# Wulizhou888/3DGS-RayTrace

Measured on AMD Instinct MI355X. Metric: Mrays/s @1080p, 1M Gaussians; achieved HBM GB/s vs peak; 1→8 GPU scaling, higher is better.
Workload: dtype f32; 1 GPU; c3: 1000000 Gaussians SH-3, 1920x1080, 4 spp, COR; gaussians=1000000, width=1920, height=1080, spp=4, sh_degree=3, parallelism=1 GPU

## Files before the change

3dgs-raytrace_amd/csrc/gsrt_render.hip:

```cpp
#include <algorithm>
#include <cmath>
#include <cstdlib>
#include <cstring>
#include <vector>
#include <type_traits>

#include "gsrt_internal.hpp"
#include "gsrt_project.hpp"

namespace gsrt {

constexpr uint32_t kStack = 512;
constexpr uint32_t kGroup = 4;
constexpr uint32_t kRCap = 128;
constexpr uint32_t kRBuf = 2 * kRCap;
constexpr uint32_t kRStack = 256;
constexpr uint32_t kGCap = 896;
#ifndef GSRT_GROUP_SEGMENTS
#define GSRT_GROUP_SEGMENTS 2
#endif
constexpr uint32_t kGSegs = GSRT_GROUP_SEGMENTS;
constexpr uint32_t kGStride = kGSegs * kGCap;
constexpr uint32_t kMoreLanes = 16;
constexpr uint32_t kGBuf = 1024;
// ... 547 lines not shown

__device__ GSRT_INLINE void add_counters(unsigned long long rays, unsigned long long cand, unsigned long long blended,
                                    unsigned long long term, unsigned long long rounds, unsigned long long restarts,
                                    unsigned long long maxc) {
    if (lane_id() != 0) return;
    unsigned long long* c = kargs().a.counters;
    atomicAdd(c + 0, rays);
    atomicAdd(c + 1, cand);
    atomicAdd(c + 2, blended);
    atomicAdd(c + 3, term);
    atomicAdd(c + 4, rounds);
    atomicAdd(c + 5, restarts);
    atomicAdd(c + 6, 1ull);
    atomicMax(c + 7, maxc);
}


struct Stage {
    SplatRec rec[kGroup];
    float sh[kGroup][3][16];
};
static_assert(sizeof(Stage) == kGroup * 256 && sizeof(Stage) % 1024 == 0, "whole wave-instructions of 16-B pieces");

template <uint32_t N>
__device__ GSRT_INLINE void wait_vmcnt() { asm volatile("s_waitcnt vmcnt(%0)" ::"n"(N) : "memory"); }
template <class V>
__device__ GSRT_INLINE void wait_stage(uint32_t younger) {
    constexpr uint32_t P = V::stage_ops;
    if (younger >= 2) wait_vmcnt<2 * P>();
    else if (younger == 1) wait_vmcnt<P>();
    else wait_vmcnt<0>();
}

__device__ GSRT_INLINE uint32_t lds_read_settled(const uint32_t* p) {
    const uint32_t a = (uint32_t)(uintptr_t)(const __attribute__((address_space(3))) uint32_t*)p;
    uint32_t v;
    asm volatile("ds_read_b32 %0, %1\n\ts_waitcnt lgkmcnt(0)" : "=v"(v) : "v"(a) : "memory");
    return v;
}

template <class V>
__device__ GSRT_INLINE void stage_issue(const uint32_t* ids, uint32_t count, uint32_t g0, uint32_t lane, Stage* dst,
                                   const SplatRec* recs, const float* sh) {
    constexpr uint32_t kRecPieces = 4 * kGroup, kPieces = V::stage_pieces, kRowPieces = V::row_pieces;
#pragma unroll
    for (uint32_t i = 0; i < (kPieces + 63) / 64; ++i) {
        const uint32_t p = i * 64 + lane;
        const bool is_rec = p < kRecPieces;
        const uint32_t q = p - kRecPieces;
        uint32_t c = g0 + (is_rec ? p >> 2 : q / kRowPieces);
        c = c < count ? c : g0;
        if (p < kPieces) {
            const uint32_t id = lds_read_settled(ids + c);
            const char* base = is_rec ? reinterpret_cast<const char*>(recs) : reinterpret_cast<const char*>(sh);
            const uint32_t stride = is_rec ? 64u : kRowPieces * 16u, off = is_rec ? (p & 3) * 16u : (q % kRowPieces) * 16u;
            __builtin_amdgcn_global_load_lds((const void*)(base + (size_t)id * stride + off),
                                             (void*)(reinterpret_cast<char*>(dst) + i * 1024), 16, 0, 0);
        }
    }
}

__device__ GSRT_INLINE void list_issue(uint32_t lt, uint32_t lane, uint32_t* ids, uint32_t* hdr) {
    const KArgs& K = kargs();
    const uint32_t* src = K.a.lists + (size_t)lt * kCap;
    __builtin_amdgcn_global_load_lds((const void*)(src + lane), (void*)ids, 4, 0, 0);
    __builtin_amdgcn_global_load_lds((const void*)(src + 64 + lane), (void*)(ids + 64), 4, 0, 0);
    if (lane < 4)
        __builtin_amdgcn_global_load_lds((const void*)(reinterpret_cast<const uint32_t*>(K.a.list_hdr + lt) + lane),
                                         (void*)hdr, 4, 0, 0);
}

template <class V>
struct CorRay {
    ObjRay R;
    float pxs, pys;
    float bs[16];
    float T, C[3];
    typename V::RayPayload k;
    bool active;
    uint32_t cand, blended, term;
#ifdef GSRT_DIAG
    uint32_t dg_staged, dg_gpass, dg_contrib, dg_blend, dg_lanes_g, dg_lanes_blend;
    uint32_t dg_stages, dg_stages_blend, dg_lane_max;
#endif
};

__device__ GSRT_INLINE float sh_channel(const float (&bs)[16], const float (&s)[16]) {
    float a = s[0];
#pragma unroll
    for (int q = 1; q < 16; ++q) a = fmaf(bs[q], s[q], a);
    return a > 0.0f ? a : 0.0f;
}
struct ShFromStage {
    const Stage* stg;
    uint32_t c;
    __device__ GSRT_INLINE void operator()(const float (&bs)[16], float (&col)[3]) const {
#pragma unroll
        for (int ch = 0; ch < 3; ++ch) {
            const float4* s4 = reinterpret_cast<const float4*>(stg->sh[c][ch]);
            const float4 q0 = s4[0], q1 = s4[1], q2 = s4[2], q3 = s4[3];
            const float s[16] = {q0.x, q0.y, q0.z, q0.w, q1.x, q1.y, q1.z, q1.w,
                                 q2.x, q2.y, q2.z, q2.w, q3.x, q3.y, q3.z, q3.w};
            col[ch] = sh_channel(bs, s);
        }
    }
};
__device__ GSRT_INLINE bool lane_of(uint64_t mask) { return __builtin_amdgcn_inverse_ballot_w64(mask); }
__device__ GSRT_INLINE const float4* feat_row(const Stage* stg, uint32_t c) {
    return reinterpret_cast<const float4*>(&stg->sh[0][0][0]) + 4 * c;
}
template <int CTRL>
__device__ GSRT_INLINE float dpp_from(float v) {
    return __int_as_float(__builtin_amdgcn_mov_dpp(__float_as_int(v), CTRL, 0xF, 0xF, false));
}
__device__ GSRT_INLINE float grad_row_sums(const float (&t)[16]) {
    const bool b3 = lane_of(0xFF00FF00FF00FF00ull), b2 = lane_of(0xF0F0F0F0F0F0F0F0ull);
    const bool b1 = lane_of(0xCCCCCCCCCCCCCCCCull), b0 = lane_of(0xAAAAAAAAAAAAAAAAull);
    float a[8], b[4], c[2];
#pragma unroll
    for (int k = 0; k < 8; ++k) a[k] = (b3 ? t[8 + k] : t[k]) + dpp_from<0x140>(b3 ? t[k] : t[8 + k]);
#pragma unroll
    for (int k = 0; k < 4; ++k) b[k] = (b2 ? a[4 + k] : a[k]) + dpp_from<0x141>(b2 ? a[k] : a[4 + k]);
#pragma unroll
    for (int k = 0; k < 2; ++k) c[k] = (b1 ? b[2 + k] : b[k]) + dpp_from<0x4E>(b1 ? b[k] : b[2 + k]);
    return (b0 ? c[1] : c[0]) + dpp_from<0xB1>(b0 ? c[0] : c[1]);
}
__device__ GSRT_INLINE float grad_stage_sums(const float (&gs)[kGroup]) {
    static_assert(kGroup == 4, "one candidate per 16-lane row");
    typedef uint32_t u32x2 __attribute__((ext_vector_type(2)));
    const u32x2 p = __builtin_amdgcn_permlane32_swap(__float_as_uint(gs[0]), __float_as_uint(gs[2]), false, false);
    const u32x2 q = __builtin_amdgcn_permlane32_swap(__float_as_uint(gs[1]), __float_as_uint(gs[3]), false, false);
    const float u = __uint_as_float(p.x) + __uint_as_float(p.y);
    const float v = __uint_as_float(q.x) + __uint_as_float(q.y);
    const u32x2 r = __builtin_amdgcn_permlane16_swap(__float_as_uint(u), __float_as_uint(v), false, false);
    return __uint_as_float(r.x) + __uint_as_float(r.y);
}
__device__ GSRT_INLINE float opgrad_stage_sums(const float (&t)[kGroup]) {
    static_assert(kGroup == 4, "one candidate per lane of a quad");
    typedef uint32_t u32x2 __attribute__((ext_vector_type(2)));
    const bool b1 = lane_of(0xCCCCCCCCCCCCCCCCull), b0 = lane_of(0xAAAAAAAAAAAAAAAAull);
    float c[2];
#pragma unroll
    for (int k = 0; k < 2; ++k) c[k] = (b1 ? t[2 + k] : t[k]) + dpp_from<0x4E>(b1 ? t[k] : t[2 + k]);
    float v = (b0 ? c[1] : c[0]) + dpp_from<0xB1>(b0 ? c[0] : c[1]);
    v = v + dpp_from<0x128>(v);
    v = v + dpp_from<0x124>(v);
    const u32x2 p = __builtin_amdgcn_permlane16_swap(__float_as_uint(v), __float_as_uint(v), false, false);
    const float u = __uint_as_float(p.x) + __uint_as_float(p.y);
    const u32x2 q = __builtin_amdgcn_permlane32_swap(__float_as_uint(u), __float_as_uint(u), false, false);
    return __uint_as_float(q.x) + __uint_as_float(q.y);
}
__device__ GSRT_INLINE float over_samples(float x, uint32_t ns) {
    const float nsf = (float)ns;
    return (ns & (ns - 1)) == 0 ? x * (1.0f / nsf) : x / nsf;
}

template <int N>
__device__ GSRT_INLINE void load_upstream(float (&G)[N], uint32_t x, uint32_t y, bool valid, uint32_t ns) {
    const KArgs& K = kargs();
    const float* gi = K.a.grad_in + ((size_t)y * K.a.width + x) * 4;
#pragma unroll
    for (int q = 0; q < N; ++q) G[q] = valid ? over_samples(gi[q], ns) : 0.0f;
}
template <uint32_t PER, class Sums, class Add>
__device__ GSRT_INLINE void flush_share(const uint32_t* ids, uint32_t mask, Sums sums, Add add) {
    const auto sum = sums();
// ... 133 lines not shown
        }
        __device__ GSRT_INLINE void flush() const {
            flush_share<1>(ids, mask, [&] { return opgrad_stage_sums(t); },
                           [&](uint32_t id, uint32_t, float sum) { atomicAdd(rows + id, sum); });
        }
    };
    __device__ GSRT_INLINE Share share(const uint32_t* ids) const { return Share{ids, rows}; }
};

enum class CorKind { plain, stats, depth, feat, grad, shgrad, opgrad };
constexpr uint32_t kFeatWaves = 4;
constexpr uint32_t kGradWaves = GSRT_GRAD_WAVES;
constexpr uint32_t kShGradWaves = GSRT_SHGRAD_WAVES;
constexpr uint32_t kOpGradWaves = GSRT_OPGRAD_WAVES;
struct NoPayload {};
struct DepthPayload { float D; };
struct ChannelPayload { float F[16]; };
template <CorKind K, bool SH, bool LUT>
struct CorVariant {
    static constexpr bool sh = SH, lut = LUT;
    static constexpr bool stats = K == CorKind::stats, depth = K == CorKind::depth;
    static constexpr bool feat = K == CorKind::feat, grad = K == CorKind::grad, shgrad = K == CorKind::shgrad;
    static constexpr bool opgrad = K == CorKind::opgrad;
    static_assert(!(feat || grad) || !SH, "feature and gradient frames evaluate no SH");
    static_assert(!shgrad || SH, "an SH gradient frame blends the SH rows");
    static constexpr uint32_t waves =
        opgrad ? kOpGradWaves : shgrad ? kShGradWaves : grad ? kGradWaves : feat ? kFeatWaves
        : SH ? (LUT ? (K == CorKind::plain ? 5 : 4) : 6) : (LUT ? 5 : 6);
    static constexpr uint32_t row_pieces = feat ? 4u : 12u;
    static constexpr uint32_t stage_pieces = SH ? 16 * kGroup : (feat ? 8 * kGroup : 4 * kGroup);
    static constexpr uint32_t stage_ops = (stage_pieces + 63) / 64;
    using Grad = std::conditional_t<grad, FeatureGrad, std::conditional_t<shgrad, ShGrad,
                                    std::conditional_t<opgrad, OpacityGrad, NoGrad>>>;
    using SumPayload = std::conditional_t<depth, DepthPayload, std::conditional_t<feat, ChannelPayload, NoPayload>>;
    using RayPayload = std::conditional_t<std::is_same_v<Grad, NoGrad>, SumPayload, typename Grad::Payload>;
};
template <class V, class Sh>
__device__ GSRT_INLINE uint64_t blend_hit(const Stage* stg, uint32_t c, float z, float alpha, uint64_t contrib,
                                          CorRay<V>& ray, Sh& grad) {
    const float tn = ray.T * (1.0f - alpha);
    const uint64_t low = __ballot(tn < 1e-4f);
    const uint64_t term = contrib & low;
    const uint64_t blend = contrib & ~low;
    if (blend) {
        float col[3] = {1.0f, 1.0f, 1.0f};
        if (V::sh) ShFromStage{stg, c}(ray.bs, col);
        grad.hit(c, blend, alpha, col, ray);
        if (lane_of(blend)) {
            const float w = alpha * ray.T;
            ray.C[0] = fmaf(col[0], w, ray.C[0]);
            if constexpr (!V::feat && !V::grad) {
                ray.C[1] = fmaf(col[1], w, ray.C[1]);
                ray.C[2] = fmaf(col[2], w, ray.C[2]);
            }
            if constexpr (V::depth) ray.k.D = fmaf(z, w, ray.k.D);
            if constexpr (V::feat) {
                const float4* frow = feat_row(stg, c);
#pragma unroll
                for (int q = 0; q < 4; ++q) {
                    const float4 f = frow[q];
                    ray.k.F[4 * q + 0] = fmaf(f.x, w, ray.k.F[4 * q + 0]);
                    ray.k.F[4 * q + 1] = fmaf(f.y, w, ray.k.F[4 * q + 1]);
                    ray.k.F[4 * q + 2] = fmaf(f.z, w, ray.k.F[4 * q + 2]);
                    ray.k.F[4 * q + 3] = fmaf(f.w, w, ray.k.F[4 * q + 3]);
                }
            }
            grad.hit_lane(c, alpha, col, ray);
            ray.T = tn;
            if (V::stats) ++ray.blended;
        }
    }
    if (term) {
        if (lane_of(term)) {
            ray.active = false;
            ray.pxs = __builtin_nanf("");
            if (V::stats) ++ray.term;
        }
    }
    return term;
}

template <class V>
constexpr bool kShPerLane = V::sh && !V::stats && !V::shgrad && !V::opgrad;
struct StageBlends {
    uint64_t blend[kGroup] = {0, 0, 0, 0};
    float w[kGroup] = {0.0f, 0.0f, 0.0f, 0.0f};
};
template <class V>
__device__ GSRT_INLINE uint64_t weigh_hit(uint32_t c, float alpha, uint64_t contrib, CorRay<V>& ray, StageBlends& sb) {
    const float tn = ray.T * (1.0f - alpha);
    const uint64_t low = __ballot(tn < 1e-4f);
    const uint64_t term = contrib & low;
    const uint64_t blend = contrib & ~low;
    sb.blend[c] = blend;
    sb.w[c] = alpha * ray.T;
    ray.T = lane_of(blend) ? tn : ray.T;
    if (term) {
        if (lane_of(term)) {
            ray.active = false;
            ray.pxs = __builtin_nanf("");
        }
    }
    return term;
}
template <class V, uint32_t J>
__device__ GSRT_INLINE bool blend_pass(const Stage* stg, const uint64_t (&at)[kGroup][kGroup], const float (&ws)[kGroup],
                                       CorRay<V>& ray) {
    uint64_t any = at[J][J];
    if constexpr (J + 1 < kGroup) any |= at[J][J + 1];
    if constexpr (J + 2 < kGroup) any |= at[J][J + 2];
    if constexpr (J + 3 < kGroup) any |= at[J][J + 3];
    if (!any) return false;
#ifdef GSRT_DIAG
    ray.dg_lane_max += 1u;
#endif
    if (lane_of(any)) {
        uint32_t cj = J;
        float w = ws[J];
        if constexpr (J + 1 < kGroup) {
            const bool here = lane_of(at[J][J + 1]);
            cj = here ? J + 1 : cj, w = here ? ws[J + 1] : w;
        }
        if constexpr (J + 2 < kGroup) {
            const bool here = lane_of(at[J][J + 2]);
            cj = here ? J + 2 : cj, w = here ? ws[J + 2] : w;
        }
        if constexpr (J + 3 < kGroup) {
            const bool here = lane_of(at[J][J + 3]);
            cj = here ? J + 3 : cj, w = here ? ws[J + 3] : w;
        }
        float col[3];
        ShFromStage{stg, cj}(ray.bs, col);
        ray.C[0] = fmaf(col[0], w, ray.C[0]);
        ray.C[1] = fmaf(col[1], w, ray.C[1]);
        ray.C[2] = fmaf(col[2], w, ray.C[2]);
        if constexpr (V::depth) ray.k.D = fmaf(stg->rec[cj].depth, w, ray.k.D);
    }
    return true;
}
template <class V>
__device__ GSRT_INLINE void blend_stage(const Stage* stg, const StageBlends& sb, CorRay<V>& ray) {
    static_assert(kGroup == 4, "two bit planes count a lane's earlier blends; blend_pass selects among four");
    if (!(sb.blend[0] | sb.blend[1] | sb.blend[2] | sb.blend[3])) return;
#ifdef GSRT_DIAG
    ray.dg_stages_blend += 1u;
#endif
    uint64_t at[kGroup][kGroup];
    uint64_t p0 = 0, p1 = 0;
#pragma unroll
    for (uint32_t c = 0; c < kGroup; ++c) {
        const uint64_t b = sb.blend[c];
        at[0][c] = b & ~p0 & ~p1;
        at[1][c] = b & p0 & ~p1;
        at[2][c] = b & ~p0 & p1;
        at[3][c] = b & p0 & p1;
        const uint64_t carry = p0 & b;
        p0 ^= b;
        p1 ^= carry;
    }
    float ws[kGroup] = {sb.w[0], sb.w[1], sb.w[2], sb.w[3]};
    asm volatile("" : "+v"(ws[0]), "+v"(ws[1]), "+v"(ws[2]), "+v"(ws[3]));
    if (!blend_pass<V, 0>(stg, at, ws, ray)) return;
    if (!blend_pass<V, 1>(stg, at, ws, ray)) return;
    if (!blend_pass<V, 2>(stg, at, ws, ray)) return;
    blend_pass<V, 3>(stg, at, ws, ray);
}

template <class V, bool FULL, class Sh>
__device__ GSRT_INLINE void shade_stage(const Stage* stg, uint32_t m, const float* lut_s, CorRay<V>& ray, Sh grad) {
    constexpr bool LUT = V::lut;
    if constexpr (!V::stats) {
        float gv[kGroup];
        uint64_t okg[kGroup];
#pragma unroll
        for (uint32_t c = 0; c < kGroup; ++c) {
            const float4 q2 = reinterpret_cast<const float4*>(&stg->rec[c])[2];
            float4 q3 = reinterpret_cast<const float4*>(&stg->rec[c])[3];
            asm volatile("" : "+v"(q3.w));
            const float c2 = q3.x, cut = LUT ? kGMax : q3.y;
            const float dx = ray.pxs - q2.x, dy = ray.pys - q2.y;
            gv[c] = fmaf(c2 * dy, dy, fmaf(q2.w * dx, dy, (q2.z * dx) * dx));
            okg[c] = (FULL || c < m) ? __ballot(__float_as_uint(gv[c]) <= __float_as_uint(cut)) : 0;
        }
#ifdef GSRT_DIAG
        ray.dg_staged += __ballot(ray.active) ? m : 0u;
        ray.dg_stages += __ballot(ray.active) ? 1u : 0u;
#endif
        [[maybe_unused]] StageBlends sb;
#pragma unroll
        for (uint32_t c = 0; c < kGroup; ++c) {
            if (!okg[c]) continue;
            float4 q0 = reinterpret_cast<const float4*>(&stg->rec[c])[0];
            const float4 q1 = reinterpret_cast<const float4*>(&stg->rec[c])[1];
            asm volatile("" : "+v"(q0.w));
            const float lo[3] = {q0.x, q0.y, q0.z}, hi[3] = {q1.x, q1.y, q1.z};
            const bool ordered = (int)__builtin_amdgcn_readfirstlane(__float_as_uint(q1.w)) >= 0;
            const uint64_t ok = okg[c] & (ordered ? __ballot(slab_hit_ordered(ray.R, lo, hi))
                                                  : __ballot(slab_hit_rel(ray.R, lo, hi)));
            const float gs = LUT ? (lane_of(ok) ? gv[c] : 0.0f) : gv[c];
            const float e = LUT ? linear_exp(lut_s, gs) : exp_neg_nocheck(-gs);
            const float a = __builtin_fminf(fabsf(q1.w) * e, 0.99f);
            const uint64_t contrib = ok & __ballot(a > kAlphaMin);
            const float alpha = lane_of(contrib) ? a : 0.0f;
#ifdef GSRT_DIAG
            ray.dg_gpass += 1u;
            ray.dg_lanes_g += (uint32_t)__popcll(okg[c]);
            ray.dg_contrib += __ballot(alpha > 0.0f) ? 1u : 0u;
            ray.dg_blend += __ballot(alpha > 0.0f && ray.T * (1.0f - alpha) >= 1e-4f) ? 1u : 0u;
            ray.dg_lanes_blend += (uint32_t)__popcll(__ballot(alpha > 0.0f && ray.T * (1.0f - alpha) >= 1e-4f));
#endif
            grad.candidate(e, fabsf(q1.w));
            uint64_t stopped;
            if constexpr (kShPerLane<V>) stopped = weigh_hit<V>(c, alpha, contrib, ray, sb);
            else stopped = blend_hit<V>(stg, c, q0.w, alpha, contrib, ray, grad);
            if (stopped) {
#pragma unroll
                for (uint32_t c1 = c + 1; c1 < kGroup; ++c1) okg[c1] &= ~stopped;
            }
        }
        if constexpr (kShPerLane<V>) blend_stage<V>(stg, sb, ray);
        if (grad.mask) grad.flush();
    } else {
        for (uint32_t c = 0; c < m; ++c) {
            const float4* r4 = reinterpret_cast<const float4*>(&stg->rec[c]);
            float4 q0 = r4[0], q1 = r4[1], q2 = r4[2], q3 = r4[3];
            asm volatile("" : "+v"(q1.w), "+v"(q2.x), "+v"(q2.y), "+v"(q2.z), "+v"(q2.w), "+v"(q3.x), "+v"(q3.z));
            float alpha = 0.0f;
            if (ray.active) {
                const float lo[3] = {q0.x, q0.y, q0.z}, hi[3] = {q1.x, q1.y, q1.z};
                if (slab_hit_rel(ray.R, lo, hi)) {
                    ++ray.cand;
                    const float dx = ray.pxs - q2.x, dy = ray.pys - q2.y;
                    const float g = fmaf(q3.x * dy, dy, fmaf(q2.w * dx, dy, (q2.z * dx) * dx));
                    if (g >= 0.0f && g <= kGMax) {
                        const float e = LUT ? linear_exp(lut_s, g) : exp_neg(-g);
                        float a = fabsf(q1.w) * e;
                        if (a > 0.99f) a = 0.99f;
                        if (a > kAlphaMin) alpha = a;
                    }
                }
            }
            blend_hit<V>(stg, c, q0.w, alpha, __ballot(alpha > 0.0f), ray, grad);
        }
    }
}


template <class V, class S>
__device__ GSRT_INLINE bool shade_sorted(const uint32_t* ids, uint32_t count, Stage* stA, Stage* stB, Stage* stC,
                             const float* lut_s, CorRay<V>& ray, const SplatRec* recs, const float* sh, S sink) {
    const uint32_t lane = lane_id();
    count = __builtin_amdgcn_readfirstlane(count);
    if (count == 0) return __ballot(ray.active) != 0;
    auto issue = [&](uint32_t g, Stage* dst) { stage_issue<V>(ids, count, g, lane, dst, recs, sh); };
    auto shade = [&](Stage* stg, uint32_t g) {
        const uint32_t m = count - g < kGroup ? count - g : kGroup;
        shade_stage<V, false>(stg, m, lut_s, ray, sink.share(ids + g));
    };
    auto shade_full = [&](Stage* stg, uint32_t g) {
        shade_stage<V, true>(stg, kGroup, lut_s, ray, sink.share(ids + g));
    };
    constexpr uint32_t kWaitTwo = 2 * V::stage_ops;
    auto wait = [count](uint32_t g) {
        wait_stage<V>((g + kGroup < count ? 1u : 0u) + (g + 2 * kGroup < count ? 1u : 0u));
    };
    issue(0, stA);
    if (kGroup < count) issue(kGroup, stB);
    bool live = true;
    uint32_t g0 = 0;
    if (!V::stats) {
        for (; g0 + 4 * kGroup < count; g0 += 3 * kGroup) {
            issue(g0 + 2 * kGroup, stC);
            wait_vmcnt<kWaitTwo>();
            shade_full(stA, g0);
            if (!__ballot(ray.active)) { live = false; break; }
            issue(g0 + 3 * kGroup, stA);
            wait_vmcnt<kWaitTwo>();
            shade_full(stB, g0 + kGroup);
            if (!__ballot(ray.active)) { live = false; break; }
            issue(g0 + 4 * kGroup, stB);
            wait_vmcnt<kWaitTwo>();
            shade_full(stC, g0 + 2 * kGroup);
            if (!__ballot(ray.active)) { live = false; break; }
        }
    }
    for (; live && g0 < count; g0 += 3 * kGroup) {
        if (g0 + 2 * kGroup < count) issue(g0 + 2 * kGroup, stC);
        wait(g0);
        shade(stA, g0);
        if (!__ballot(ray.active)) { live = false; break; }
        const uint32_t g1 = g0 + kGroup;
        if (g1 >= count) break;
        if (g1 + 2 * kGroup < count) issue(g1 + 2 * kGroup, stA);
        wait(g1);
        shade(stB, g1);
        if (!__ballot(ray.active)) { live = false; break; }
        const uint32_t g2 = g1 + kGroup;
        if (g2 >= count) break;
        if (g2 + 2 * kGroup < count) issue(g2 + 2 * kGroup, stB);
        wait(g2);
        shade(stC, g2);
        if (!__ballot(ray.active)) { live = false; break; }
    }
// ... 409 lines not shown
        p.valid = p.x < kargs().a.width && p.y < kargs().a.height;
        return p;
    }
    __device__ GSRT_INLINE TileRect rect_here() const {
        uint32_t tx = x0 >> lgtw, ty = y0 >> lgth;
        asm volatile("" : "+s"(tx), "+s"(ty));
        return tile_rect(tx, ty, tw, th);
    }
};

template <class V>
struct PixelSums {
    float rgba[4];
    typename V::SumPayload k;
    template <class Op>
    __device__ GSRT_INLINE void each(Op op) {
#pragma unroll
        for (int q = 0; q < 4; ++q) op(rgba[q]);
        if constexpr (V::depth) op(k.D);
        if constexpr (V::feat) {
#pragma unroll
            for (int q = 0; q < 16; ++q) op(k.F[q]);
        }
    }
    template <class Op>
    __device__ GSRT_INLINE void each_extra_at(size_t pix, Op op) {
        if constexpr (V::depth) op(k.D, kargs().a.depth_out + pix);
        if constexpr (V::feat) {
            const uint32_t C = kargs().a.feat_channels;
            float* of = kargs().a.feat_out + pix * C;
#pragma unroll
            for (int q = 0; q < 16; ++q)
                if ((uint32_t)q < C) op(k.F[q], of + q);
        }
    }
    template <class Op>
    __device__ GSRT_INLINE void each_at(float* colour, size_t pix, Op op) {
#pragma unroll
        for (int q = 0; q < 4; ++q) op(rgba[q], colour + q);
        each_extra_at(pix, op);
    }
    __device__ GSRT_INLINE void take(const CorRay<V>& ray) {
        constexpr bool grey = V::feat || V::grad;
        rgba[0] = ray.C[0]; rgba[1] = ray.C[grey ? 0 : 1]; rgba[2] = ray.C[grey ? 0 : 2]; rgba[3] = 1.0f - ray.T;
        if constexpr (V::depth) k.D = ray.k.D;
        if constexpr (V::feat) {
#pragma unroll
            for (int q = 0; q < 16; ++q) k.F[q] = ray.k.F[q];
        }
    }
};

template <class V>
__device__ GSRT_INLINE CorRay<V> cor_ray(const CorTile::Pixel& p, uint32_t S, uint32_t pass, uint32_t passes) {
    CorRay<V> ray;
    {
        const KArgs& K = kargs();
        const uint32_t sidx = pass * S + p.s;
        uint32_t seed = K.ubo.random_seed;
        for (uint32_t q = 0; q < sidx; ++q) { random_float(&seed); random_float(&seed); }
        const float jx = random_float(&seed);
        const float jy = random_float(&seed);
        ray.pxs = (float)p.x + jx;
        ray.pys = (float)p.y + jy;
        float o[3], d[3];
        gen_ray(K.ubo, ray.pxs, ray.pys, o, d);
        ray.R = make_obj_ray(d);
        if (V::sh) sh_basis(d, ray.bs);
    }
    ray.T = 1.0f;
    ray.C[0] = ray.C[1] = ray.C[2] = 0.0f;
    if constexpr (V::depth) ray.k.D = 0.0f;
    if constexpr (V::feat) {
#pragma unroll
        for (int q = 0; q < 16; ++q) ray.k.F[q] = 0.0f;
    }
    V::Grad::load(ray.k, p.x, p.y, p.valid, S * passes);
    ray.active = p.valid;
    if (!p.valid) ray.pxs = __builtin_nanf("");
    ray.cand = ray.blended = ray.term = 0;
#ifdef GSRT_DIAG
    ray.dg_staged = ray.dg_gpass = ray.dg_contrib = ray.dg_blend = ray.dg_lanes_g = ray.dg_lanes_blend = 0;
    ray.dg_stages = ray.dg_stages_blend = ray.dg_lane_max = 0;
#endif
    return ray;
}

__device__ GSRT_INLINE Collected round_from_list(const CorTile& t, bool& prefetched, uint32_t* ids, const uint32_t* lhdr,
                                                 uint64_t& lo, uint32_t& gpos) {
    Collected cl{};
    if (!prefetched) list_issue(t.lt, lane_here(), ids, const_cast<uint32_t*>(lhdr));
    prefetched = false;
    __syncthreads();
    const uint4 h = make_uint4(lhdr[0], lhdr[1], lhdr[2], lhdr[3]);
    const uint32_t* src = kargs().a.lists + (size_t)t.lt * kCap;
    cl.count = h.x & 0x7fffffffu;
    cl.more = (h.x >> 31) != 0;
    for (uint32_t i = 128u + lane_here(); i < cl.count; i += 64) ids[i] = src[i];
    cl.total = cl.count;
    lo = ((uint64_t)h.w << 32) | h.z;
    gpos = h.y;
    __syncthreads();
    return cl;
}
__device__ GSRT_INLINE Collected round_from_group(const CorTile& t, uint32_t* ids, uint64_t& lo, uint32_t& gpos, bool& found) {
    Collected cl{};
    const KArgs& K = kargs();
    const uint32_t g = (t.y0 / t.th / K.a.fg) * K.a.groups_x + (t.x0 / t.tw / K.a.fg);
    const uint4 gh = K.a.ghdr[g];
    const uint32_t gcount = gh.x & 0x7fffffffu;
    found = gpos < gcount;
    if (!found) return cl;
    const uint64_t* gl = K.a.glist + (size_t)g * kGStride;
    const float4* fps = K.a.footprint;
    const TileRect rect_c = t.rect_here();
    uint32_t out = 0;
    while (gpos < gcount && out < kCap) {
        const uint32_t i = gpos + lane_here();
        bool keep = false;
        uint64_t key = 0;
        if (i < gcount) {
            key = gl[i];
            keep = fp_meets(fps, (uint32_t)key, rect_c);
        }
        const uint64_t b = __ballot(keep);
        const uint32_t rank = popc_below(b), n = (uint32_t)__popcll(b), room = kCap - out;
        if (keep && rank < room) ids[out + rank] = (uint32_t)key;
        if (n > room) {
            const uint64_t kb = __ballot(keep && rank < room);
            gpos += (uint32_t)(63 - __builtin_clzll(kb)) + 1u;
            out = kCap;
        } else {
            gpos = gpos + 64u < gcount ? gpos + 64u : gcount;
            out += n;
        }
    }
    cl.count = cl.total = out;
    cl.more = gpos < gcount || (gh.x >> 31) != 0;
    lo = gl[gpos - 1];
    __syncthreads();
    return cl;
}
template <class V>
__device__ GSRT_INLINE Collected round_from_traversal(const CorTile& t, uint64_t* keys, uint32_t* stack, uint32_t* ids,
                                                      uint64_t& lo, bool has_lo, uint32_t& restarts) {
    const uint32_t lim = kargs().a.stack_limit < kRStack ? kargs().a.stack_limit : kRStack;
    const Collected cl = collect_robust<kRCap, kRBuf>(t.rect_here(), lo, has_lo, keys, stack, KeyCorRec{}, restarts,
                                                      !V::stats && kargs().a.cull2d, lim, FrontRegs{}, !V::stats);
    lo = cl.count ? keys[cl.count - 1] : lo;
    const uint32_t ln = lane_here();
    for (uint32_t base = 0; base < cl.count; base += 64) {
        const uint32_t i = base + ln;
        const uint32_t v = i < cl.count ? (uint32_t)keys[i] : 0u;
        asm volatile("" ::: "memory");
        if (i < cl.count) ids[i] = v;
        asm volatile("" ::: "memory");
    }
    __syncthreads();
    return cl;
}

template <class V>
__global__ __launch_bounds__(64) __attribute__((amdgpu_waves_per_eu(V::waves)))
void k_render_cor(const KArgs karg) {
    union CorLds {
        struct { uint64_t keys[kRBuf]; uint32_t stack[kRStack]; } t;
// ... 36 lines not shown
    tile.lt = __builtin_amdgcn_readfirstlane(tile.lt);
    bool prefetched = false;
    if (kargs().a.prelisted) {
        list_issue(tile.lt, lane, ids, lhdr);
        prefetched = true;
    }
    tile.x0 = __builtin_amdgcn_readfirstlane(tile.x0);
    tile.y0 = __builtin_amdgcn_readfirstlane(tile.y0);
    tile.lgS = (uint32_t)__builtin_ctz(tile.S);
    tile.lgtw = (uint32_t)__builtin_ctz(tile.tw); tile.lgth = (uint32_t)__builtin_ctz(tile.th);
    const uint32_t S = tile.S;
    PixelSums<V> sums{};
    uint32_t st_cand = 0, st_blend = 0, st_term = 0, st_rounds = 0, restarts = 0, maxc = 0;
#ifdef GSRT_DIAG
    unsigned long long diag_collect = 0, diag_shade = 0;
#endif
    for (uint32_t pass = 0; pass < passes; ++pass) {
        CorRay<V> ray = cor_ray<V>(tile.pixel(), S, pass, passes);
        [[maybe_unused]] uint32_t sweep = 0;
        do {
            uint64_t lo = 0;
            bool has_lo = false;
            uint32_t gpos = 0;
            for (;;) {
#ifdef GSRT_DIAG
                const unsigned long long d0 = __builtin_amdgcn_s_memtime();
                if (!has_lo) diag_setup += d0 - (pass == 0 ? diag_entry : diag_last);
#endif
                Collected cl;
                bool listed = true;
                if (kargs().a.prelisted && !has_lo) {
                    cl = round_from_list(tile, prefetched, ids, lhdr, lo, gpos);
                } else {
                    listed = false;
                    if (kargs().a.use_groups) cl = round_from_group(tile, ids, lo, gpos, listed);
                }
                if (!listed) cl = round_from_traversal<V>(tile, keys, stack, ids, lo, has_lo, restarts);
#ifdef GSRT_DIAG
                const unsigned long long d1 = __builtin_amdgcn_s_memtime();
                diag_collect += d1 - d0;
#endif
                ++st_rounds;
                if (cl.total > maxc) maxc = cl.total;
                const bool live = V::opgrad && sweep == 0
                    ? shade_sorted<V>(ids, cl.count, &stA, &stB, &stC, lut_s, ray, recs, shp, NoGrad{})
                    : shade_sorted<V>(ids, cl.count, &stA, &stB, &stC, lut_s, ray, recs, shp, V::Grad::of_frame());
#ifdef GSRT_DIAG
                diag_last = __builtin_amdgcn_s_memtime();
                diag_shade += diag_last - d1;
#endif
                if (!cl.more || !live) break;
                has_lo = true;
                __syncthreads();
            }
            if constexpr (V::opgrad) {
                if (sweep == 0) {
                    sums.take(ray);
                    const float fin[4] = {ray.C[0], ray.C[1], ray.C[2], ray.T};
                    ray = cor_ray<V>(tile.pixel(), S, pass, passes);
#pragma unroll
                    for (int q = 0; q < 4; ++q) ray.k.fin[q] = fin[q];
                }
            }
        } while (V::opgrad && ++sweep < 2);
        if constexpr (!V::opgrad) sums.take(ray);
        if (passes > 1) {
            const CorTile::Pixel p = tile.pixel();
            if (p.valid) {
                const KArgs& K = kargs();
                const size_t pix = (size_t)p.y * K.a.width + p.x;
                float4* o = (K.a.dump8 ? K.a.accum : reinterpret_cast<float4*>(K.a.out)) +
                            (K.a.packed ? (size_t)tile.lt * (tile.tw * tile.th) + p.in_tile : pix);
                if (pass > 0) sums.each_at(&o->x, pix, [](float& v, const float* home) { v = *home + v; });
                if (pass + 1 < passes) sums.each_at(&o->x, pix, [](float v, float* home) { *home = v; });
            }
        }
        st_cand += ray.cand; st_blend += ray.blended; st_term += ray.term;
#ifdef GSRT_DIAG
        if (!V::stats && lane == 0) {
            const uint32_t dg[6] = {ray.dg_staged, ray.dg_gpass, ray.dg_contrib, ray.dg_blend, ray.dg_lanes_g, ray.dg_lanes_blend};
            for (int q = 0; q < 6; ++q) atomicAdd(kargs().a.counters + 16 + q, (unsigned long long)dg[q]);
            const uint32_t ds[3] = {ray.dg_stages, ray.dg_stages_blend, ray.dg_lane_max};
            for (int q = 0; q < 3; ++q) atomicAdd(kargs().a.counters + 25 + q, (unsigned long long)ds[q]);
        }
#endif
    }
    if (S > 1) sums.each([](float& v) { v = v + dpp_from<0xB1>(v); });
    if (S > 2) sums.each([](float& v) { v = v + dpp_from<0x4E>(v); });
    for (uint32_t off = 4; off < S; off <<= 1) sums.each([off](float& v) { v = v + __shfl_xor(v, (int)off); });
    for (uint32_t off = 1; V::stats && off < S; off <<= 1) {
        st_cand += __shfl_xor(st_cand, (int)off);
        st_blend += __shfl_xor(st_blend, (int)off);
        st_term += __shfl_xor(st_term, (int)off);
    }
    const KArgs& K = kargs();
    const uint32_t ns = S * passes;
    const CorTile::Pixel p = tile.pixel();
    if (p.valid && p.s == 0) {
        sums.each([ns](float& v) { v = over_samples(v, ns); });
        const float4 v = make_float4(sums.rgba[0], sums.rgba[1], sums.rgba[2], sums.rgba[3]);
        const size_t pix = (size_t)p.y * K.a.width + p.x;
        const size_t idx = K.a.packed ? (size_t)tile.lt * (tile.tw * tile.th) + p.in_tile : pix;
        if (K.a.dump8) {
            const uint32_t code = dump8_code(v);
            reinterpret_cast<uint32_t*>(K.a.out)[idx] = code;
            if (code & kDump8Escape) {
                const uint32_t e = atomicAdd(&K.a.esc[0].x, 1u);
                if (e < K.a.esc_cap)
                    K.a.esc[1 + e] = make_uint4((uint32_t)idx, __float_as_uint(v.x), __float_as_uint(v.y), __float_as_uint(v.z));
            }
        } else {
            reinterpret_cast<float4*>(K.a.out)[idx] = v;
        }
        sums.each_extra_at(pix, [](float x, float* home) { *home = x; });
        if (V::stats && K.a.ray_stats)
            reinterpret_cast<uint4*>(K.a.ray_stats)[pix] = make_uint4(st_cand, st_blend, st_rounds, st_term);
    }
#ifdef GSRT_DIAG
    if (lane == 0) {
        atomicAdd(K.a.counters + 9, diag_collect);
        atomicAdd(K.a.counters + 10, diag_shade);
        const unsigned long long dend = __builtin_amdgcn_s_memtime();
        atomicAdd(K.a.counters + 11, dend - diag_entry);
        atomicAdd(K.a.counters + 1, diag_setup);
        atomicAdd(K.a.counters + 2, dend - diag_last);
    }
#endif
    if (K.a.tile_cost && lane == 0) K.a.tile_cost[tile.lt] = (uint32_t)__builtin_amdgcn_s_memrealtime() - t_tile0;
    if (V::stats) {
        const uint32_t lead = (p.valid && p.s == 0) ? 1u : 0u;
        add_counters(wave_sum(p.valid ? 1u : 0u) * passes, wave_sum(lead ? st_cand : 0u), wave_sum(lead ? st_blend : 0u),
                     wave_sum(lead ? st_term : 0u), st_rounds, restarts, maxc);
    }
    GSRT_WT_END(0, tile.lt);
}


template <bool STATS>
__global__ __launch_bounds__(64) void k_render_ref(const KArgs karg) {
    __shared__ uint64_t keys[2 * kCap];
    __shared__ uint32_t stack[kStack];
    __shared__ float lut_s[512];
    (void)karg;
    const uint32_t lane = lane_id();
    {
        const float* lut = kargs().a.lut;
        for (uint32_t i = lane; i < 512; i += 64) lut_s[i] = lut[i];
    }
    __syncthreads();
    uint32_t lt, x0, y0, samples, bounces;
    {
        const KArgs& K = kargs();
        const uint32_t t = blockIdx.x;
        if (t >= K.a.ntiles_local) return;
        lt = xcd_local_tile(t, K.a.ntiles_local);
        uint32_t tx, ty;
        band_tile(lt, K.a.row0, K.a.row1, K.a.tiles_x, tx, ty);
        x0 = tx * 8; y0 = ty * 8;
        samples = K.a.samples; bounces = K.a.bounces;
    }
    const uint32_t px = x0 + (lane & 7u), py = y0 + (lane >> 3);
    bool valid;
    float o[3];
    ObjRay R;
    float tri = kTMax;
    {
// ... 840 lines not shown
```

profiles/diag_split.py:

```python
import os
import sys

ROOT = os.path.dirname(os.path.dirname(os.path.abspath(__file__)))
sys.path.insert(0, os.path.join(ROOT, "3dgs-raytrace_amd"))
import gsrt

cfg = sys.argv[1] if len(sys.argv) > 1 else "c3"
n, W, H, spp, with_sh = {"c3": (1_000_000, 1920, 1080, 4, True), "c2": (100_000, 1920, 1080, 1, False),
                          "c4": (1_000_000, 3840, 2160, 1, False), "c5": (5_000_000, 1920, 1080, 16, False)}[cfg]
ctx = gsrt.Context(0)
c, r, s, o, sh = gsrt.synth_cloud(gsrt.SYNTH_COR, n, 42, with_sh)
sc = gsrt.Scene.from_model(ctx, c, r, s, o, sh)
sc.build_bvh()
ubo = gsrt.camera_from_modelview(gsrt.lookat((0, 0, 0), (0, 0, -1)), 60.0, W, H, 1.0, spp, 16)
share = bool(os.environ.get("GSRT_DEBUG_RANK_OF"))
if share:
    ctx.comm_init_loopback()
for _ in range(3):
    (sc.render_sharded_async if share else sc.render_async)(ubo, gsrt.MODE_COR)
ctx.synchronize()
if share:
    sc.render_sharded(ubo, gsrt.MODE_COR, want_image=False)
else:
    sc.render(ubo, gsrt.MODE_COR)
cnt = ctx.debug_counters()
col, sha, tot = int(cnt[9]), int(cnt[10]), int(cnt[11])
print(f"{cfg}: wave-cycles collect(traversal+sort) {col / tot:.3f}  shade {sha / tot:.3f}  other {(tot - col - sha) / tot:.3f}"
      f"  (sum of per-wave s_memtime, {tot / 1e9:.2f} G)")
print(f"{cfg}: collect() wave-cycles traversal {int(cnt[12]) / 1e9:.3f} G, final cull+sort {int(cnt[13]) / 1e9:.3f} G; "
      f"steps {int(cnt[14])}, popped nodes {int(cnt[15])} (per tile: {int(cnt[14]) / (W * H * spp / 64):.1f} steps, {int(cnt[15]) / (W * H * spp / 64):.0f} nodes)")
print(f"{cfg}: k_group_list wave-cycles {int(cnt[6]) / 1e9:.3f} G, of which tile filter {int(cnt[7]) / 1e9:.3f} G; "
      f"groups with an overflowing list: {int(cnt[5])}; group list length max {int(cnt[4])}, sum {int(cnt[3])}")
ng = max(int(cnt[3]) and 1, 1)
print(f"{cfg}: k_group_list tile filter split: per-lane tile tests (incl. the chunk's footprint loads) "
      f"{int(cnt[22]) / 1e9:.3f} G, per-tile list output {int(cnt[23]) / 1e9:.3f} G; group list to HBM {int(cnt[24]) / 1e9:.3f} G")
print(f"{cfg}: wave-cycles from entry: tile+ray setup {int(cnt[1]) / tot:.3f}, reduction+store tail {int(cnt[2]) / tot:.3f}")
waves = W * H * spp / 64
st, gp, co, bl, lg, lb = (int(x) for x in cnt[16:22])
print(f"{cfg}: per wave: staged candidates {st / waves:.1f}, some lane passes g {gp / waves:.1f}, some lane alpha > 0 "
      f"{co / waves:.1f}, some lane blends (SH) {bl / waves:.1f}; lanes per g-survivor {lg / max(gp, 1):.1f}, "
      f"lanes per blending candidate {lb / max(bl, 1):.1f}")
ns, nb, lm = (int(x) for x in cnt[25:28])
if nb:
    print(f"{cfg}: stages shaded {ns} ({ns / waves:.2f} per wave), with a blend {nb}; per shaded stage E {bl / ns:.3f} "
          f"E' {lm / ns:.3f}; per stage with a blend E {bl / nb:.3f} E' {lm / nb:.3f}; E'/E {lm / max(bl, 1):.3f}")
```

Baseline: 6529 Mrays/s.

## Compact per-lane candidate shading: run slab/alpha/SH per lane pass after gaussian test

For the SH per-lane path, the slab test, exponent, alpha and blend are no longer evaluated once per candidate across the wave. After the gaussian g-test, each lane's surviving candidates are ranked with bit planes and processed in up to four lane passes. Each pass handles one candidate per lane, selected dynamically, so the slab/exp/SH work runs only about max-per-lane times instead of once per candidate with any surviving lane. In exchange, candidate records are loaded with per-lane indices rather than uniform ones, and the slab ordering becomes a divergent choice. Diagnostic counters and the profiling script are extended to measure this.

```diff
diff --git a/3dgs-raytrace_amd/csrc/gsrt_render.hip b/3dgs-raytrace_amd/csrc/gsrt_render.hip
--- a/3dgs-raytrace_amd/csrc/gsrt_render.hip
+++ b/3dgs-raytrace_amd/csrc/gsrt_render.hip
@@ -653,6 +653,7 @@
 #ifdef GSRT_DIAG
     uint32_t dg_staged, dg_gpass, dg_contrib, dg_blend, dg_lanes_g, dg_lanes_blend;
     uint32_t dg_stages, dg_stages_blend, dg_lane_max;
+    uint32_t dg_g_any, dg_g_lane_max;
 #endif
 };
 
@@ -952,66 +953,75 @@
 
 template <class V>
 constexpr bool kShPerLane = V::sh && !V::stats && !V::shgrad && !V::opgrad;
-struct StageBlends {
-    uint64_t blend[kGroup] = {0, 0, 0, 0};
-    float w[kGroup] = {0.0f, 0.0f, 0.0f, 0.0f};
-};
-template <class V>
-__device__ GSRT_INLINE uint64_t weigh_hit(uint32_t c, float alpha, uint64_t contrib, CorRay<V>& ray, StageBlends& sb) {
+template <class V, uint32_t J>
+__device__ GSRT_INLINE bool lane_pass(const Stage* stg, const uint64_t (&at)[kGroup][kGroup], const float (&gv)[kGroup],
+                                      uint64_t& gone, const float* lut_s, CorRay<V>& ray) {
+    constexpr bool LUT = V::lut;
+    uint64_t any = at[J][J];
+    if constexpr (J + 1 < kGroup) any |= at[J][J + 1];
+    if constexpr (J + 2 < kGroup) any |= at[J][J + 2];
+    if constexpr (J + 3 < kGroup) any |= at[J][J + 3];
+    any &= ~gone;
+    if (!any) return false;
+    uint32_t cj = J;
+    float g = gv[J];
+    if constexpr (J + 1 < kGroup) {
+        const bool here = lane_of(at[J][J + 1]);
+        cj = here ? J + 1 : cj, g = here ? gv[J + 1] : g;
+    }
+    if constexpr (J + 2 < kGroup) {
+        const bool here = lane_of(at[J][J + 2]);
+        cj = here ? J + 2 : cj, g = here ? gv[J + 2] : g;
+    }
+    if constexpr (J + 3 < kGroup) {
+        const bool here = lane_of(at[J][J + 3]);
+        cj = here ? J + 3 : cj, g = here ? gv[J + 3] : g;
+    }
+    float4 q0 = reinterpret_cast<const float4*>(&stg->rec[cj])[0];
+    const float4 q1 = reinterpret_cast<const float4*>(&stg->rec[cj])[1];
+    asm volatile("" : "+v"(q0.w));
+    const float lo[3] = {q0.x, q0.y, q0.z}, hi[3] = {q1.x, q1.y, q1.z};
+    const uint64_t general = any & __ballot((int)__float_as_uint(q1.w) < 0);
+    const uint64_t ok = any & (general ? __ballot(slab_hit_rel(ray.R, lo, hi)) : __ballot(slab_hit_ordered(ray.R, lo, hi)));
+    const float gs = LUT ? (lane_of(ok) ? g : 0.0f) : g;
+    const float e = LUT ? linear_exp(lut_s, gs) : exp_neg_nocheck(-gs);
+    const float alpha = __builtin_fminf(fabsf(q1.w) * e, 0.99f);
+    const uint64_t contrib = ok & __ballot(alpha > kAlphaMin);
     const float tn = ray.T * (1.0f - alpha);
     const uint64_t low = __ballot(tn < 1e-4f);
     const uint64_t term = contrib & low;
     const uint64_t blend = contrib & ~low;
-    sb.blend[c] = blend;
-    sb.w[c] = alpha * ray.T;
-    ray.T = lane_of(blend) ? tn : ray.T;
+#ifdef GSRT_DIAG
+    ray.dg_lane_max += 1u;
+    ray.dg_lanes_g += (uint32_t)__popcll(any);
+    ray.dg_lanes_blend += (uint32_t)__popcll(blend);
+#endif
+    if (blend) {
+        if (lane_of(blend)) {
+            float col[3];
+            ShFromStage{stg, cj}(ray.bs, col);
+            const float w = alpha * ray.T;
+            ray.C[0] = fmaf(col[0], w, ray.C[0]);
+            ray.C[1] = fmaf(col[1], w, ray.C[1]);
+            ray.C[2] = fmaf(col[2], w, ray.C[2]);
+            if constexpr (V::depth) ray.k.D = fmaf(q0.w, w, ray.k.D);
+            ray.T = tn;
+        }
+    }
     if (term) {
         if (lane_of(term)) {
             ray.active = false;
             ray.pxs = __builtin_nanf("");
         }
-    }
-    return term;
-}
-template <class V, uint32_t J>
-__device__ GSRT_INLINE bool blend_pass(const Stage* stg, const uint64_t (&at)[kGroup][kGroup], const float (&ws)[kGroup],
-                                       CorRay<V>& ray) {
-    uint64_t any = at[J][J];
-    if constexpr (J + 1 < kGroup) any |= at[J][J + 1];
-    if constexpr (J + 2 < kGroup) any |= at[J][J + 2];
-    if constexpr (J + 3 < kGroup) any |= at[J][J + 3];
-    if (!any) return false;
-#ifdef GSRT_DIAG
-    ray.dg_lane_max += 1u;
-#endif
-    if (lane_of(any)) {
-        uint32_t cj = J;
-        float w = ws[J];
-        if constexpr (J + 1 < kGroup) {
-            const bool here = lane_of(at[J][J + 1]);
-            cj = here ? J + 1 : cj, w = here ? ws[J + 1] : w;
-        }
-        if constexpr (J + 2 < kGroup) {
-            const bool here = lane_of(at[J][J + 2]);
-            cj = here ? J + 2 : cj, w = here ? ws[J + 2] : w;
-        }
-        if constexpr (J + 3 < kGroup) {
-            const bool here = lane_of(at[J][J + 3]);
-            cj = here ? J + 3 : cj, w = here ? ws[J + 3] : w;
-        }
-        float col[3];
-        ShFromStage{stg, cj}(ray.bs, col);
-        ray.C[0] = fmaf(col[0], w, ray.C[0]);
-        ray.C[1] = fmaf(col[1], w, ray.C[1]);
-        ray.C[2] = fmaf(col[2], w, ray.C[2]);
-        if constexpr (V::depth) ray.k.D = fmaf(stg->rec[cj].depth, w, ray.k.D);
+        gone |= term;
     }
     return true;
 }
 template <class V>
-__device__ GSRT_INLINE void blend_stage(const Stage* stg, const StageBlends& sb, CorRay<V>& ray) {
-    static_assert(kGroup == 4, "two bit planes count a lane's earlier blends; blend_pass selects among four");
-    if (!(sb.blend[0] | sb.blend[1] | sb.blend[2] | sb.blend[3])) return;
+__device__ GSRT_INLINE void shade_lanes(const Stage* stg, const uint64_t (&okg)[kGroup], const float (&gv)[kGroup],
+                                        const float* lut_s, CorRay<V>& ray) {
+    static_assert(kGroup == 4, "two bit planes count a lane's earlier candidates; lane_pass selects among four");
+    if (!(okg[0] | okg[1] | okg[2] | okg[3])) return;
 #ifdef GSRT_DIAG
     ray.dg_stages_blend += 1u;
 #endif
@@ -1019,7 +1029,7 @@
     uint64_t p0 = 0, p1 = 0;
 #pragma unroll
     for (uint32_t c = 0; c < kGroup; ++c) {
-        const uint64_t b = sb.blend[c];
+        const uint64_t b = okg[c];
         at[0][c] = b & ~p0 & ~p1;
         at[1][c] = b & p0 & ~p1;
         at[2][c] = b & ~p0 & p1;
@@ -1028,12 +1038,11 @@
         p0 ^= b;
         p1 ^= carry;
     }
-    float ws[kGroup] = {sb.w[0], sb.w[1], sb.w[2], sb.w[3]};
-    asm volatile("" : "+v"(ws[0]), "+v"(ws[1]), "+v"(ws[2]), "+v"(ws[3]));
-    if (!blend_pass<V, 0>(stg, at, ws, ray)) return;
-    if (!blend_pass<V, 1>(stg, at, ws, ray)) return;
-    if (!blend_pass<V, 2>(stg, at, ws, ray)) return;
-    blend_pass<V, 3>(stg, at, ws, ray);
+    uint64_t gone = 0;
+    if (!lane_pass<V, 0>(stg, at, gv, gone, lut_s, ray)) return;
+    if (!lane_pass<V, 1>(stg, at, gv, gone, lut_s, ray)) return;
+    if (!lane_pass<V, 2>(stg, at, gv, gone, lut_s, ray)) return;
+    lane_pass<V, 3>(stg, at, gv, gone, lut_s, ray);
 }
 
 template <class V, bool FULL, class Sh>
@@ -1055,8 +1064,16 @@
 #ifdef GSRT_DIAG
         ray.dg_staged += __ballot(ray.active) ? m : 0u;
         ray.dg_stages += __ballot(ray.active) ? 1u : 0u;
-#endif
-        [[maybe_unused]] StageBlends sb;
+        if (__ballot(ray.active)) {
+            const uint64_t two = (okg[0] & okg[1]) | (okg[2] & okg[3]) | ((okg[0] | okg[1]) & (okg[2] | okg[3]));
+            const uint64_t three = (okg[0] & okg[1] & (okg[2] | okg[3])) | (okg[2] & okg[3] & (okg[0] | okg[1]));
+            ray.dg_g_any += (okg[0] ? 1u : 0u) + (okg[1] ? 1u : 0u) + (okg[2] ? 1u : 0u) + (okg[3] ? 1u : 0u);
+            ray.dg_g_lane_max += (okg[0] & okg[1] & okg[2] & okg[3]) ? 4u : three ? 3u : two ? 2u
+                                 : (okg[0] | okg[1] | okg[2] | okg[3]) ? 1u : 0u;
+        }
+#endif
+        if constexpr (kShPerLane<V>) shade_lanes<V>(stg, okg, gv, lut_s, ray);
+        else
 #pragma unroll
         for (uint32_t c = 0; c < kGroup; ++c) {
             if (!okg[c]) continue;
@@ -1080,15 +1097,12 @@
             ray.dg_lanes_blend += (uint32_t)__popcll(__ballot(alpha > 0.0f && ray.T * (1.0f - alpha) >= 1e-4f));
 #endif
             grad.candidate(e, fabsf(q1.w));
-            uint64_t stopped;
-            if constexpr (kShPerLane<V>) stopped = weigh_hit<V>(c, alpha, contrib, ray, sb);
-            else stopped = blend_hit<V>(stg, c, q0.w, alpha, contrib, ray, grad);
+            const uint64_t stopped = blend_hit<V>(stg, c, q0.w, alpha, contrib, ray, grad);
             if (stopped) {
 #pragma unroll
                 for (uint32_t c1 = c + 1; c1 < kGroup; ++c1) okg[c1] &= ~stopped;
             }
         }
-        if constexpr (kShPerLane<V>) blend_stage<V>(stg, sb, ray);
         if (grad.mask) grad.flush();
     } else {
         for (uint32_t c = 0; c < m; ++c) {
@@ -1664,6 +1678,7 @@
 #ifdef GSRT_DIAG
     ray.dg_staged = ray.dg_gpass = ray.dg_contrib = ray.dg_blend = ray.dg_lanes_g = ray.dg_lanes_blend = 0;
     ray.dg_stages = ray.dg_stages_blend = ray.dg_lane_max = 0;
+    ray.dg_g_any = ray.dg_g_lane_max = 0;
 #endif
     return ray;
 }
@@ -1866,6 +1881,8 @@
             for (int q = 0; q < 6; ++q) atomicAdd(kargs().a.counters + 16 + q, (unsigned long long)dg[q]);
             const uint32_t ds[3] = {ray.dg_stages, ray.dg_stages_blend, ray.dg_lane_max};
             for (int q = 0; q < 3; ++q) atomicAdd(kargs().a.counters + 25 + q, (unsigned long long)ds[q]);
+            atomicAdd(kargs().a.counters + 30, (unsigned long long)ray.dg_g_any);
+            atomicAdd(kargs().a.counters + 31, (unsigned long long)ray.dg_g_lane_max);
         }
 #endif
     }
diff --git a/profiles/diag_split.py b/profiles/diag_split.py
--- a/profiles/diag_split.py
+++ b/profiles/diag_split.py
@@ -37,10 +37,16 @@
 print(f"{cfg}: wave-cycles from entry: tile+ray setup {int(cnt[1]) / tot:.3f}, reduction+store tail {int(cnt[2]) / tot:.3f}")
 waves = W * H * spp / 64
 st, gp, co, bl, lg, lb = (int(x) for x in cnt[16:22])
-print(f"{cfg}: per wave: staged candidates {st / waves:.1f}, some lane passes g {gp / waves:.1f}, some lane alpha > 0 "
-      f"{co / waves:.1f}, some lane blends (SH) {bl / waves:.1f}; lanes per g-survivor {lg / max(gp, 1):.1f}, "
-      f"lanes per blending candidate {lb / max(bl, 1):.1f}")
 ns, nb, lm = (int(x) for x in cnt[25:28])
-if nb:
-    print(f"{cfg}: stages shaded {ns} ({ns / waves:.2f} per wave), with a blend {nb}; per shaded stage E {bl / ns:.3f} "
-          f"E' {lm / ns:.3f}; per stage with a blend E {bl / nb:.3f} E' {lm / nb:.3f}; E'/E {lm / max(bl, 1):.3f}")
+if gp:
+    print(f"{cfg}: per wave: staged candidates {st / waves:.1f}, some lane passes g {gp / waves:.1f}, some lane alpha > 0 "
+          f"{co / waves:.1f}, some lane blends {bl / waves:.1f}; lanes per g-survivor {lg / max(gp, 1):.1f}, "
+          f"lanes per blending candidate {lb / max(bl, 1):.1f}")
+elif lm:
+    print(f"{cfg}: per wave: staged candidates {st / waves:.1f}, passes run {lm / waves:.1f}; lanes per pass {lg / lm:.1f}, "
+          f"blending lanes per pass {lb / lm:.1f}")
+    print(f"{cfg}: stages shaded {ns} ({ns / waves:.2f} per wave), with a lane passing g {nb}; passes per shaded stage "
+          f"{lm / ns:.3f}")
+eg, egl = int(cnt[30]), int(cnt[31])
+if ns and eg:
+    print(f"{cfg}: per shaded stage E_g {eg / ns:.3f} E'_g {egl / ns:.3f}; E'_g/E_g {egl / eg:.3f}")
```

After: 6713 Mrays/s, median of 6. +2.8%, better.
